# connortannahill/MM-ADMM

Hardware: AMD Instinct MI355X
Metric: ADMM iterations/sec on 1M-node 2D mesh; achieved HBM GB/s in SpMV (higher is better)
Workload: dtype f64

## Files before the change

### include/mmx_sparse.h

```cpp
#ifndef MMX_SPARSE_H
#define MMX_SPARSE_H

#include <stdint.h>

#include "mmadmm.h"

#ifdef __cplusplus
extern "C" {
#endif

typedef struct mmx_param_iter {
  int order;
  int level;
  int drop_ilu;
  int ipiv;
  int iscal;
  int nitmax;
  double resid_reduc;
  int info;
  double drop_tol;
  int new_rhat;
  int iaccel;
  int north;
} mmx_param_iter;

typedef struct mmx_struc_s* mmx_struc;
typedef struct mmx_matrix_s* mmx_matrix;

typedef struct mmx_sparse_stats {
  long long solves, iterations, spmvs, sweeps, factors;
  double t_spmv_ms, t_sweep_ms, t_factor_ms, t_vec_ms, t_solve_ms;
  long long n_spmv_timed, n_sweep_timed, n_factor_timed;
  double spmv_bytes;
  double last_rms, rmsi;
  int sweep_mode;
  int sweep_e;
  int factor_mode;
  int sweep_e_bwd;
} mmx_sparse_stats;

void mmx_param_iter_default(mmx_param_iter* p);
void mmx_param_iter_mesh(mmx_param_iter* p);

int mmx_struc_create(int n, int no_diag, mmx_struc* out);
int mmx_struc_set_entry(mmx_struc s, int row, int col);
int mmx_struc_set_entries(mmx_struc s, long long count, const int32_t* rows, const int32_t* cols);
int mmx_struc_mesh_pattern(mmx_struc s, int dim, int nF, const int32_t* F);
int mmx_struc_pack(mmx_struc s);
int mmx_struc_get(mmx_struc s, int* n, long long* nnz, int32_t* ia, int32_t* ja);
int mmx_struc_destroy(mmx_struc s);

int mmx_matrix_create(int device, int n, const int32_t* ia, const int32_t* ja, mmx_matrix* out);
int mmx_matrix_create_from_struc(int device, mmx_struc s, mmx_matrix* out);
int mmx_matrix_sizes(mmx_matrix m, int* n, long long* nnz);
int mmx_matrix_stream(mmx_matrix m, void** hip_stream);
int mmx_matrix_set_values(mmx_matrix m, const double* a);
int mmx_matrix_set_values_device(mmx_matrix m, const double* d_a);
int mmx_matrix_set_rhs(mmx_matrix m, const double* b);
int mmx_matrix_set_rhs_device(mmx_matrix m, const double* d_b);
int mmx_matrix_set_toler(mmx_matrix m, const double* tol);
int mmx_matrix_sfac(mmx_matrix m, const mmx_param_iter* p);
int mmx_matrix_solve(mmx_matrix m, const mmx_param_iter* p, double* x, int* nitr, int initial_guess);
int mmx_matrix_solve_device(mmx_matrix m, const mmx_param_iter* p, double* d_x, int* nitr, int initial_guess);
int mmx_matrix_matmult(mmx_matrix m, const double* x, double* y);
int mmx_matrix_matmult_device(mmx_matrix m, const double* d_x, double* d_y);
int mmx_matrix_factor(mmx_matrix m);
int mmx_matrix_ilu_solve(mmx_matrix m, const double* b, double* x);
int mmx_matrix_ilu_solve_device(mmx_matrix m, const double* d_b, double* d_x);
int mmx_matrix_factor_nnz(mmx_matrix m, long long* nnzf);
int mmx_matrix_get_factor(mmx_matrix m, int32_t* iaf, int32_t* jaf, double* af, int32_t* diag);
int mmx_matrix_get_scale(mmx_matrix m, double* scal);
int mmx_matrix_set_timing(mmx_matrix m, int on);
int mmx_matrix_stats_get(mmx_matrix m, mmx_sparse_stats* out);
int mmx_matrix_stats_reset(mmx_matrix m);
int mmx_matrix_destroy(mmx_matrix m);

int mmx_ilu_symbolic(int n, const int32_t* ia, const int32_t* ja, int level, long long* nnzf, int32_t* iaf,
                     int32_t* jaf, int32_t* diag);

int mmx_matrix_chain_prof(mmx_matrix m, unsigned long long* out, int reset);
int mmx_sweep_schedule_info(int n, const int32_t* ia, const int32_t* ja, int level, int fwd, long long* info);
int mmx_factor_schedule_info(int n, const int32_t* ia, const int32_t* ja, int level, long long* info);

int mmx_stream_copy(int device, const double* d_src, double* d_dst, long long n, int reps, int variant, double* ms);
int mmx_occupy(int device, int blocks, double ms);
int mmx_occupy_wait(void);

#ifdef __cplusplus
}
#endif
#endif
```

### mm-admm_amd/csrc/host/sparse.cpp

```cpp
#include <omp.h>

#include <algorithm>
#include <chrono>
#include <climits>
#include <cmath>
#include <cstdio>
#include <cstring>
#include <exception>
#include <string>
#include <thread>
#include <queue>
#include <vector>

#include "../../../include/mmx_sparse.h"
#include "../kernels/sparse_kernels.h"
#include "chain_sched.h"
#include "common.h"

namespace mmx {
namespace {

struct PhaseTimer {
  bool on;
  const char* who;
// ... 141 lines not shown
      rl[i][q] = lev[cols[q]];
      lev[cols[q]] = kAbsent;
    }
    if (dgRel[i] < 0) throw Error(MMADMM_ERR_INVALID, "row " + std::to_string(i) + " has no diagonal entry");
  }
  iaf.assign(n + 1, 0);
  for (int i = 0; i < n; ++i) iaf[i + 1] = iaf[i] + (int)rj[i].size();
  jaf.resize(iaf[n]);
  for (int i = 0; i < n; ++i) std::copy(rj[i].begin(), rj[i].end(), jaf.begin() + iaf[i]);
}

namespace {

int spmv_version() {
  static int v = [] {
    const char* e = getenv("MMX_SPMV");
    return (e && atoi(e) == 1) ? 1 : 2;
  }();
  return v;
}

void check_params(const mmx_param_iter& p) {
  if (p.order != 0) throw Error(MMADMM_ERR_INVALID, "unsupported ParamIter.order (only natural ordering, 0)");
  if (p.drop_ilu != 0) throw Error(MMADMM_ERR_INVALID, "unsupported ParamIter.drop_ilu (only level-of-fill ILU, 0)");
  if (p.ipiv != 0) throw Error(MMADMM_ERR_INVALID, "unsupported ParamIter.ipiv (only no pivoting, 0)");
  if (p.iscal != 0 && p.iscal != 1)
    throw Error(MMADMM_ERR_INVALID, "unsupported ParamIter.iscal (0 no scaling, 1 diagonal row scaling)");
  if (p.iaccel != 0 && p.iaccel != 1 && p.iaccel != -1)
    throw Error(MMADMM_ERR_INVALID, "unsupported ParamIter.iaccel (0 CG-STAB, 1 ORTHOMIN, -1 CG)");
  if (p.iaccel == 1 && p.north < 1) throw Error(MMADMM_ERR_INVALID, "ParamIter.north must be >= 1 for ORTHOMIN");
  if (p.level < 0) throw Error(MMADMM_ERR_INVALID, "ParamIter.level must be >= 0");
}

struct Timer {
  hipEvent_t a = nullptr, b = nullptr;
  bool armed = false;
  void init() {
    if (!a) {
      MMX_HIP(hipEventCreateWithFlags(&a, hipEventDisableSystemFence));
      MMX_HIP(hipEventCreateWithFlags(&b, hipEventDisableSystemFence));
    }
  }
  ~Timer() {
    if (a) (void)hipEventDestroy(a);
    if (b) (void)hipEventDestroy(b);
  }
};

}

struct SparseMatrix {
  int device = 0;
  hipStream_t st = nullptr;
  int n = 0;
  long long nnz = 0;
  std::vector<int> ia, ja;
  DevBuf<int> d_ia, d_ja, d_rowblk;
  DevBuf<int4> d_desc;
  int nblk = 0;
  DevBuf<double> d_a, d_b, d_tol;
  bool tolSet = false;
  bool symbolic = false;
  int level = -1;
  std::vector<int> iaf, jaf, dgRel;
  DevBuf<int> d_iaf, d_jaf, d_dg, d_amap, d_permf, d_permb;
  DevBuf<int2> d_piv;
  DevBuf<int> d_toff;
  DevBuf<signed char> d_tgt;
  bool facLds = false;
  int nchf = 0, nchb = 0, nlevf = 0, nlevb = 0;
  DevBuf<double> d_af;
  DevBuf<unsigned> d_flags, d_ctl;
  DevBuf<uint64_t> d_gy, d_gx;
  unsigned epoch = 0, fepoch = 0;
  struct ChainDir {
    int E = 0;
    long long nent = 0, nslot = 0;
    DevBuf<int> bandSlot, bandT, bandImp, bandNImp, bandE, bandOrder, laneStart, laneLen, laneSkew, laneNs, code, src, dsrc,
        impRow, impSlot, impWait, impNeed;
    DevBuf<uint16_t> code16;
    DevBuf<double> val, dval;
    ChainArgs args{};
  };
  ChainDir chf, chb;
  bool useChain = false;
  struct FactorDir {
    DevBuf<int> bandSlot, bandT, laneLen, laneSkew, bandOrder, bandImp, bandNImp, impPos, impCnt, impSlot, impWait,
        impNeed, meta, rowStart, vsrc;
    DevBuf<uint16_t> code;
    DevBuf<double> val, af0;
    DevBuf<uint64_t> gU;
    FactorArgs args{};
// ... 15 lines not shown
  int ominNorth = 0;
  DevBuf<AccelScalars> d_asc;
  AccelScalars* h_asc = nullptr;
  bool timing = false;
  mmx_sparse_stats stats{};
  Timer tm[4];

  SparseMatrix(int dev, int n_, const int* ia_, const int* ja_) : device(dev), n(n_) {
    if (n <= 0) throw Error(MMADMM_ERR_INVALID, "matrix size must be positive");
    if (ia_[0] != 0) throw Error(MMADMM_ERR_INVALID, "ia[0] must be 0");
    for (int i = 0; i < n; ++i)
      if (ia_[i + 1] < ia_[i]) throw Error(MMADMM_ERR_INVALID, "ia must be non-decreasing");
    nnz = ia_[n];
    int bad = 0;
#pragma omp parallel for schedule(static) reduction(max : bad)
    for (long long k = 0; k < nnz; ++k)
      if (ja_[k] < 0 || ja_[k] >= n) bad = 1;
    if (bad) throw Error(MMADMM_ERR_INVALID, "column index out of range");
    ia.assign(ia_, ia_ + n + 1);
    ja.resize(nnz);
#pragma omp parallel for schedule(static)
    for (long long k = 0; k < nnz; ++k) ja[k] = ja_[k];
    int ndev = 0;
    if (hipGetDeviceCount(&ndev) != hipSuccess || ndev == 0) throw Error(MMADMM_ERR_HIP, "no HIP device available");
    MMX_HIP(hipSetDevice(device));
    MMX_HIP(hipStreamCreateWithFlags(&st, hipStreamNonBlocking));
    d_ia.upload(ia.data(), ia.size(), st);
    d_ja.alloc((size_t)nnz + 2);
    if (nnz * sizeof(int) >= ((size_t)16 << 20))
      upload_staged(d_ja.p, ja.data(), (size_t)nnz * sizeof(int), st);
    else if (nnz)
      MMX_HIP(hipMemcpyAsync(d_ja.p, ja.data(), (size_t)nnz * sizeof(int), hipMemcpyHostToDevice, st));
    MMX_HIP(hipMemsetAsync(d_ja.p + nnz, 0, 2 * sizeof(int), st));
    d_a.alloc(nnz + 2);
    MMX_HIP(hipMemsetAsync(d_a.p, 0, sizeof(double) * (nnz + 2), st));
    d_b.alloc(n);
    MMX_HIP(hipMemsetAsync(d_b.p, 0, sizeof(double) * n, st));
    std::vector<int> rb{0};
    int r0 = 0;
    while (r0 < n) {
      int r = r0 + 1;
      while (r < n && ia[r + 1] - ia[r0] <= kSpmvTile && r - r0 < 4 * kSpmvBlock) ++r;
      rb.push_back(r);
      r0 = r;
    }
    nblk = (int)rb.size() - 1;
    d_rowblk.upload(rb.data(), rb.size(), st);
    std::vector<int4> desc(nblk);
    for (int b = 0; b < nblk; ++b) desc[b] = make_int4(rb[b], rb[b + 1], ia[rb[b]], ia[rb[b + 1]]);
    d_desc.upload(desc.data(), desc.size(), st);
    std::vector<int> adiag(n, -1);
    int missing = 0;
#pragma omp parallel for schedule(static) reduction(max : missing)
    for (int i = 0; i < n; ++i) {
      for (int k = ia[i]; k < ia[i + 1]; ++k)
        if (ja[k] == i) {
          adiag[i] = k;
          break;
        }
      if (adiag[i] < 0) missing = 1;
    }
    allDiag = missing == 0;
    d_adiag.upload(adiag.data(), adiag.size(), st);
    MMX_HIP(hipStreamSynchronize(st));
    for (DevBuf<double>* v : {&d_res, &d_res0, &d_p, &d_vbar, &d_avbar, &d_s, &d_z, &d_t, &d_x, &d_tmp}) v->alloc(n);
    d_part.alloc((size_t)std::max(nblk, vec_grid(n)) * 3);
    d_sc.alloc(1);
    MMX_HIP(hipMemsetAsync(d_sc.p, 0, sizeof(CgsScalars), st));
    MMX_HIP(hipHostMalloc((void**)&h_sc, sizeof(CgsScalars), hipHostMallocDefault));
    d_asc.alloc(1);
    MMX_HIP(hipMemsetAsync(d_asc.p, 0, sizeof(AccelScalars), st));
    MMX_HIP(hipHostMalloc((void**)&h_asc, sizeof(AccelScalars), hipHostMallocDefault));
    d_ctl.alloc(16);
    MMX_HIP(hipMemsetAsync(d_ctl.p, 0, 16 * sizeof(unsigned), st));
    d_gy.alloc(2 * (size_t)n);
    d_gx.alloc(2 * (size_t)n);
    MMX_HIP(hipMemsetAsync(d_gy.p, 0, 16 * (size_t)n, st));
    MMX_HIP(hipMemsetAsync(d_gx.p, 0, 16 * (size_t)n, st));
    d_flags.alloc(n);
    MMX_HIP(hipMemsetAsync(d_flags.p, 0, sizeof(unsigned) * n, st));
    stats.spmv_bytes = 12.0 * (double)nnz + 4.0 * (n + 1) + 16.0 * n;
    MMX_HIP(hipStreamSynchronize(st));
  }
  ~SparseMatrix() {
    if (st) (void)hipStreamSynchronize(st);
    if (evSpin) (void)hipEventDestroy(evSpin);
    if (h_sc) (void)hipHostFree(h_sc);
    if (h_asc) (void)hipHostFree(h_asc);
    if (st) (void)hipStreamDestroy(st);
  }

  hipEvent_t evSpin = nullptr;
  void spin_sync() {
    static const bool spin = [] {
      const char* e = getenv("MMX_SPIN");
      return !(e && atoi(e) == 0);
    }();
    if (!spin) {
      MMX_HIP(hipStreamSynchronize(st));
      return;
    }
    if (!evSpin) MMX_HIP(hipEventCreateWithFlags(&evSpin, hipEventDisableTiming));
    MMX_HIP(hipEventRecord(evSpin, st));
    hipError_t r;
    while ((r = hipEventQuery(evSpin)) == hipErrorNotReady) __builtin_ia32_pause();
    MMX_HIP(r);
  }

  unsigned* tickets() { return d_ctl.p; }
  unsigned* errw() { return d_ctl.p + 8; }

  void sfac(const mmx_param_iter& p) {
    check_params(p);
    PhaseTimer pt("sfac");
    symbolic_ilu(n, ia, ja, p.level, iaf, jaf, dgRel);
    pt.mark("symbolic");
// ... 388 lines not shown

  void ilu_apply(int pro, const double* src, double* p, double* out, unsigned* tk) {
    begin(1);
    const unsigned ey = next_epoch();
    if (useChain)
      launch_chain_sweep(true, pro, chf.E, chf.args, src, p, d_res.p, d_avbar.p, d_sc.p, nullptr, d_gy.p, nullptr, ey,
                         tk, errw(), st);
    else
      launch_sweep(true, pro, d_iaf.p, d_jaf.p, d_dg.p, d_af.p, d_permf.p, nchf, src, p, d_res.p, d_avbar.p, d_sc.p,
                   nullptr, d_gy.p, nullptr, ey, tk, errw(), st);
    const unsigned ex = next_epoch();
    const char* bg = getenv("MMX_BWD_GRAN");
    const bool fromGran = !(bg && atoi(bg) == 0);
    if (useChain) {
      launch_chain_sweep(false, 0, chb.E, chb.args, nullptr, nullptr, nullptr, nullptr, nullptr, d_gy.p, d_gx.p,
                         fromGran ? nullptr : out, ex, tk + 1, errw(), st);
      if (fromGran) launch_gran_extract(n, d_gx.p, out, st);
    } else
      launch_sweep(false, 0, d_iaf.p, d_jaf.p, d_dg.p, d_af.p, d_permb.p, nchb, nullptr, nullptr, nullptr, nullptr,
                   nullptr, d_gy.p, d_gx.p, out, ex, tk + 1, errw(), st);
    MMX_HIP(hipGetLastError());
    const float ms = end(1);
    stats.sweeps += 2;
    if (timing) {
      stats.t_sweep_ms += ms;
      stats.n_sweep_timed += 2;
    }
  }

  void spmv(int epi, const double* x, double* y, const double* e1) {
    begin(0);
    if (spmv_version() == 1)
      launch_spmv(epi, nblk, d_rowblk.p, d_ia.p, d_ja.p, d_a.p, x, y, e1, d_part.p, st);
    else
      launch_spmv2(epi, nblk, d_desc.p, d_ia.p, d_ja.p, d_a.p, x, y, e1, d_part.p, st);
    MMX_HIP(hipGetLastError());
    const float ms = end(0);
    stats.spmvs++;
    if (timing) {
      stats.t_spmv_ms += ms;
      stats.n_spmv_timed++;
    }
  }

  void scale_rows() {
    if (!allDiag) throw Error(MMADMM_ERR_INVALID, "ParamIter.iscal = 1 needs a diagonal entry in every row");
    if (!d_ascal.p) d_ascal.alloc(n);
    launch_scale_rows(nblk, d_desc.p, d_ia.p, d_adiag.p, d_a.p, d_b.p, d_ascal.p, st);
    MMX_HIP(hipGetLastError());
    scaled = true;
    if (scaledVersion != valVersion) {
      scaledVersion = valVersion;
      factVersion = -1;
    }
  }

  void omin_buffers(int north) {
    if (ominNorth == north) return;
    ominNorth = 0;
    try {
      d_oq.alloc((size_t)north * n);
      d_oaq.alloc((size_t)north * n);
      d_oms.alloc(2 * (size_t)north);
      d_opart.alloc((size_t)std::max(north, 2) * vec_grid(n));
    } catch (...) {
      (void)hipGetLastError();
      d_oq.alloc(0);
      d_oaq.alloc(0);
// ... 508 lines not shown
  return guarded([&] {
    MMX_M(m);
    if (!M.symbolic) throw Error(MMADMM_ERR_INVALID, "no symbolic factor (call mmx_matrix_sfac)");
    if (iaf) std::memcpy(iaf, M.iaf.data(), sizeof(int) * (M.n + 1));
    if (jaf) std::memcpy(jaf, M.jaf.data(), sizeof(int) * M.jaf.size());
    if (diag) std::memcpy(diag, M.dgRel.data(), sizeof(int) * M.n);
    if (af) {
      MMX_HIP(hipMemcpyAsync(af, M.d_af.p, sizeof(double) * M.jaf.size(), hipMemcpyDeviceToHost, M.st));
      MMX_HIP(hipStreamSynchronize(M.st));
    }
  });
}

int mmx_matrix_get_scale(mmx_matrix m, double* scal) {
  return guarded([&] {
    MMX_M(m);
    if (!scal) throw Error(MMADMM_ERR_INVALID, "bad arguments");
    if (!M.scaled) {
      std::fill(scal, scal + M.n, 1.0);
      return;
    }
    MMX_HIP(hipMemcpyAsync(scal, M.d_ascal.p, sizeof(double) * M.n, hipMemcpyDeviceToHost, M.st));
    MMX_HIP(hipStreamSynchronize(M.st));
  });
}

int mmx_matrix_set_timing(mmx_matrix m, int on) {
  return guarded([&] {
    MMX_M(m);
    M.timing = on != 0;
  });
}

int mmx_matrix_stats_get(mmx_matrix m, mmx_sparse_stats* out) {
  return guarded([&] {
    MMX_M(m);
    if (out) {
      *out = M.stats;
      out->sweep_mode = M.useChain ? 1 : 0;
      out->factor_mode = M.useChainFactor ? 1 : M.facWave ? 2 : 0;
      out->sweep_e = M.useChain ? M.chf.E : 0;
      out->sweep_e_bwd = M.useChain ? M.chb.E : 0;
    }
  });
}

int mmx_matrix_chain_prof(mmx_matrix m, unsigned long long* out, int reset) {
  return guarded([&] {
    MMX_M(m);
    if (!M.d_cprof.p) throw Error(MMADMM_ERR_INVALID, "chain profiling off (set MMX_CHAIN_PROF=1 before sfac)");
    if (out)
      MMX_HIP(hipMemcpyAsync(out, M.d_cprof.p, 1024 * sizeof(unsigned long long), hipMemcpyDeviceToHost, M.st));
    if (reset) MMX_HIP(hipMemsetAsync(M.d_cprof.p, 0, 1024 * sizeof(unsigned long long), M.st));
    MMX_HIP(hipStreamSynchronize(M.st));
  });
}

int mmx_matrix_stats_reset(mmx_matrix m) {
  return guarded([&] {
    MMX_M(m);
    const double bytes = M.stats.spmv_bytes;
    M.stats = mmx_sparse_stats{};
    M.stats.spmv_bytes = bytes;
  });
}

int mmx_ilu_symbolic(int n, const int32_t* ia, const int32_t* ja, int level, long long* nnzf, int32_t* iaf,
                     int32_t* jaf, int32_t* diag) {
  return guarded([&] {
    if (n <= 0 || !ia || !ja || level < 0) throw Error(MMADMM_ERR_INVALID, "bad arguments");
    std::vector<int> via(ia, ia + n + 1), vja(ja, ja + ia[n]), fia, fja, dg;
    mmx::symbolic_ilu(n, via, vja, level, fia, fja, dg);
    if (nnzf) *nnzf = (long long)fja.size();
    if (iaf) std::memcpy(iaf, fia.data(), sizeof(int) * (n + 1));
    if (jaf) std::memcpy(jaf, fja.data(), sizeof(int) * fja.size());
// ... 107 lines not shown
```

### mm-admm_amd/csrc/kernels/layout.h

```cpp
#pragma once

#ifndef MMX_ZU_INTER
#define MMX_ZU_INTER 0
#endif
#ifndef MMX_SPMV_TILE
#define MMX_SPMV_TILE 2048
#endif
#ifndef MMX_SPMV_BLOCK
#define MMX_SPMV_BLOCK 256
#endif
#ifndef MMX_B3_PAIRS
#define MMX_B3_PAIRS 1
#endif
#ifndef MMX_CHAIN_VEC
#define MMX_CHAIN_VEC 1
#endif
#ifndef MMX_CHAIN_CODE16
#define MMX_CHAIN_CODE16 1
#endif

namespace mmx {
constexpr unsigned kLayoutPartials = 6;
constexpr unsigned kLayoutBkinvBlock = 64;
constexpr unsigned kLayoutWord = 0x4d000000u | ((unsigned)(MMX_ZU_INTER != 0) << 0) |
                                 ((unsigned)(MMX_CHAIN_VEC != 0) << 1) | ((unsigned)(MMX_CHAIN_CODE16 != 0) << 2) |
                                 (((unsigned)MMX_SPMV_TILE / 256u & 0xFu) << 4) |
                                 (((unsigned)MMX_SPMV_BLOCK / 64u & 0xFu) << 8) | ((kLayoutPartials & 0xFu) << 12) |
                                 ((kLayoutBkinvBlock / 64u & 0x3u) << 16) | ((unsigned)(MMX_B3_PAIRS != 0) << 18);
}
```

### mm-admm_amd/csrc/kernels/sparse_kernels.h

```cpp
#pragma once
#include <hip/hip_runtime.h>
#include <stdint.h>

#include "layout.h"

namespace mmx {

constexpr int kSpmvTile = MMX_SPMV_TILE;
constexpr int kSpmvBlock = MMX_SPMV_BLOCK;
constexpr int kSweepRows = 64;
constexpr int kSweepGrid = 128;
constexpr int kVecBlock = 256;
int vec_grid(int n);

struct CgsScalars {
  double rho, rholst, alpha, omega, beta, rmsi, rms, ctol, iconv;
  int conv;
  int pad;
};

struct SweepCtl {
  unsigned* tickets;
  unsigned* err;
};

void launch_spmv(int epi, int nblk, const int* rowblk, const int* ia, const int* ja, const double* a,
                 const double* x, double* y, const double* e1, double* partials, hipStream_t st);
void launch_spmv2(int epi, int nblk, const int4* desc, const int* ia, const int* ja, const double* a,
                  const double* x, double* y, const double* e1, double* partials, hipStream_t st);

void launch_ilu_factor(const int* ia, const int* ja, const double* a, const int* amap, const int* iaf, const int* jaf,
                       const int* dg, const int2* piv, const int* perm, int nchunks, double* af, unsigned* flags,
                       unsigned epoch, unsigned* ticket, unsigned* err, hipStream_t st);

constexpr int kFacW = 127;
void launch_ilu_factor_lds(const int* ia, const double* a, const int* amap, const int* iaf, const int* jaf, const int* dg,
                           const int2* piv, const int* toff, const signed char* tgt, const int* perm, int nchunks,
                           double* af, unsigned* flags, unsigned epoch, unsigned* ticket, unsigned* err, hipStream_t st);

constexpr int kFacWaveNL = 32;
void launch_ilu_factor_wave(const int* ia, const double* a, const int* amap, const int* iaf, const int* dg,
                            const int2* piv, const int* jaf, const int* toff, const signed char* tgt, const int* perm,
                            int nrows, double* af, unsigned* flags, uint64_t* gF, unsigned epoch, unsigned* ticket,
                            unsigned* err, hipStream_t st);
void launch_fac_prep(int n, const int* iaf, const int* jaf, const int* dg, const long long* rowTot, int2* piv,
                     int* toff, signed char* tgt, hipStream_t st);
void launch_occupy(int blocks, double ms, double* sink, hipStream_t st);

void launch_sweep(bool fwd, int pro, const int* iaf, const int* jaf, const int* dg, const double* af, const int* perm,
                  int nchunks, const double* src, double* p, const double* res, const double* avbar, const CgsScalars* sc,
                  const uint64_t* gin, uint64_t* gout, double* out, unsigned epoch, unsigned* ticket, unsigned* err,
                  hipStream_t st);

inline constexpr bool chain_code16(int ee) { return MMX_CHAIN_CODE16 || ee > 32; }

struct ChainArgs {
  const int* bandSlot;
  const int* bandT;
  const int* bandImp;
  const int* bandNImp;
  const int* laneStart;
  const int* laneLen;
// ... 84 lines not shown
```

### mm-admm_amd/csrc/kernels/sparse_kernels.hip

```cpp
#include <hip/hip_runtime.h>

#include <algorithm>

#include <cstdlib>

#include "block_reduce.h"
#include "sparse_kernels.h"

namespace mmx {

namespace {

constexpr unsigned kSpinMax = 1u << 24;
constexpr int kBatch = 4;
constexpr int kFactorBatch = 8;

__device__ __forceinline__ void store_granule(uint64_t* g, unsigned epoch, double v) {
  const uint64_t bits = (uint64_t)__double_as_longlong(v);
  const uint64_t tag = (uint64_t)epoch << 32;
  __hip_atomic_store(g, tag | (bits & 0xffffffffull), __ATOMIC_RELAXED, __HIP_MEMORY_SCOPE_AGENT);
  __hip_atomic_store(g + 1, tag | (bits >> 32), __ATOMIC_RELAXED, __HIP_MEMORY_SCOPE_AGENT);
}

__device__ __forceinline__ bool load_granule(const uint64_t* g, unsigned epoch, double& v) {
// ... 73 lines not shown
        pv[1] += s * s;
      }
    }
  } else {
    double s = 0.0;
    for (int c = k0; c < k1; c += kSpmvTile) {
      const int ce = (c + kSpmvTile < k1) ? c + kSpmvTile : k1;
      for (int k = c + (int)threadIdx.x; k < ce; k += kSpmvBlock) prod[k - c] = a[k] * x[ja[k]];
      __syncthreads();
      if (threadIdx.x == 0)
        for (int k = c; k < ce; ++k) s += prod[k - c];
      __syncthreads();
    }
    if (threadIdx.x == 0) {
      y[r0] = s;
      if (EPI == 1) pv[0] += e1[r0] * s;
      if (EPI == 2) {
        pv[0] += s * e1[r0];
        pv[1] += s * s;
      }
    }
  }
  if (EPI != 0) {
    __syncthreads();
    block_sum<2, kSpmvBlock>(pv, red);
    if (threadIdx.x == 0) {
      partials[(size_t)b * 2 + 0] = pv[0];
      partials[(size_t)b * 2 + 1] = pv[1];
    }
  }
}

constexpr int kSpmvPairs = kSpmvTile / (2 * kSpmvBlock) + 1;
typedef int v2i_t __attribute__((ext_vector_type(2)));
typedef double v2d_t __attribute__((ext_vector_type(2)));

template <int EPI>
__global__ void __launch_bounds__(kSpmvBlock) k_spmv2(const int4* __restrict__ desc, int nblk,
                                                       const int* __restrict__ ia, const int* __restrict__ ja,
                                                       const double* __restrict__ a, const double* __restrict__ x,
                                                       double* __restrict__ y, const double* __restrict__ e1,
                                                       double* __restrict__ partials) {
  __shared__ double prod[kSpmvTile + 2];
  __shared__ double red[kSpmvBlock][2];
  const int G = (int)gridDim.x;
  const int b = (int)(blockIdx.x % 8) * (G / 8) + (int)(blockIdx.x / 8);
  if (b >= nblk) return;
  const int tid = (int)threadIdx.x;
  const int4 d = desc[b];
  const int r0 = d.x, r1 = d.y, k0 = d.z, k1 = d.w;
  double pv[2] = {0.0, 0.0};
  if (k1 - k0 <= kSpmvTile) {
    const int ka = k0 & ~1;
    const int np = (k1 - ka + 1) >> 1;
    const int rf = r0 + tid;
    const int rc = rf < r1 ? rf : r1 - 1;
    int ib = ia[rc], ie = ia[rc + 1];
    double ef = 0.0;
    if (EPI != 0) ef = e1[rc];
    const int pmax = np > 0 ? np - 1 : 0;
    v2i_t jv[kSpmvPairs];
    v2d_t av[kSpmvPairs];
#pragma unroll
    for (int j = 0; j < kSpmvPairs; ++j) {
      const int p = min(tid + j * kSpmvBlock, pmax);
      jv[j] = __builtin_nontemporal_load(reinterpret_cast<const v2i_t*>(ja + ka) + p);
      av[j] = __builtin_nontemporal_load(reinterpret_cast<const v2d_t*>(a + ka) + p);
    }
    double xv0[kSpmvPairs], xv1[kSpmvPairs];
#pragma unroll
    for (int j = 0; j < kSpmvPairs; ++j) {
      xv0[j] = x[jv[j].x];
      xv1[j] = x[jv[j].y];
    }
#pragma unroll
    for (int j = 0; j < kSpmvPairs; ++j) {
      const int p = tid + j * kSpmvBlock;
      if (p < np) {
        prod[2 * p] = av[j].x * xv0[j];
        prod[2 * p + 1] = av[j].y * xv1[j];
      }
    }
    __syncthreads();
    for (int r = rf; r < r1; r += kSpmvBlock) {
      if (r != rf) {
        ib = ia[r];
        ie = ia[r + 1];
        if (EPI != 0) ef = e1[r];
      }
      double s = 0.0;
      for (int kk = ib; kk < ie; ++kk) s += prod[kk - ka];
      y[r] = s;
      if (EPI == 1) pv[0] += ef * s;
      if (EPI == 2) {
        pv[0] += s * ef;
        pv[1] += s * s;
      }
    }
  } else {
    double s = 0.0;
    for (int c = k0; c < k1; c += kSpmvTile) {
      const int ce = (c + kSpmvTile < k1) ? c + kSpmvTile : k1;
      for (int k = c + tid; k < ce; k += kSpmvBlock) prod[k - c] = a[k] * x[ja[k]];
      __syncthreads();
      if (tid == 0)
        for (int k = c; k < ce; ++k) s += prod[k - c];
      __syncthreads();
    }
    if (tid == 0) {
      y[r0] = s;
      if (EPI == 1) pv[0] += e1[r0] * s;
      if (EPI == 2) {
        pv[0] += s * e1[r0];
        pv[1] += s * s;
      }
// ... 535 lines not shown
    sc->rho = rho;
    sc->beta = beta;
    sc->rholst = rho;
    sc->conv = 0;
  } else if (MODE == 1) {
    sc->alpha = sc->rho / v[0];
  } else if (MODE == 2) {
    sc->omega = v[0] / (v[1] + tiny);
  } else {
    const double rms = sqrt(v[0]);
    sc->rms = rms;
    sc->iconv = v[2];
    sc->conv = (v[2] == 0.0 || (rms / sc->rmsi) < sc->ctol) ? 1 : 0;
    const double rho = v[1];
    double beta = rho / (sc->rholst + tiny);
    beta *= (sc->alpha / (sc->omega + tiny));
    sc->rho = rho;
    sc->beta = beta;
    sc->rholst = rho;
  }
}

void launch_spmv(int epi, int nblk, const int* rowblk, const int* ia, const int* ja, const double* a, const double* x,
                 double* y, const double* e1, double* partials, hipStream_t st) {
  if (nblk <= 0) return;
  if (epi == 0)
    hipLaunchKernelGGL(k_spmv<0>, dim3(nblk), dim3(kSpmvBlock), 0, st, rowblk, ia, ja, a, x, y, e1, partials);
  else if (epi == 1)
    hipLaunchKernelGGL(k_spmv<1>, dim3(nblk), dim3(kSpmvBlock), 0, st, rowblk, ia, ja, a, x, y, e1, partials);
  else
    hipLaunchKernelGGL(k_spmv<2>, dim3(nblk), dim3(kSpmvBlock), 0, st, rowblk, ia, ja, a, x, y, e1, partials);
}

void launch_spmv2(int epi, int nblk, const int4* desc, const int* ia, const int* ja, const double* a, const double* x,
                  double* y, const double* e1, double* partials, hipStream_t st) {
  if (nblk <= 0) return;
  const dim3 g((unsigned)((nblk + 7) / 8 * 8)), bl(kSpmvBlock);
  if (epi == 0)
    hipLaunchKernelGGL(k_spmv2<0>, g, bl, 0, st, desc, nblk, ia, ja, a, x, y, e1, partials);
  else if (epi == 1)
    hipLaunchKernelGGL(k_spmv2<1>, g, bl, 0, st, desc, nblk, ia, ja, a, x, y, e1, partials);
  else
    hipLaunchKernelGGL(k_spmv2<2>, g, bl, 0, st, desc, nblk, ia, ja, a, x, y, e1, partials);
}

void launch_ilu_factor_lds(const int* ia, const double* a, const int* amap, const int* iaf, const int* jaf, const int* dg,
                           const int2* piv, const int* toff, const signed char* tgt, const int* perm, int nchunks,
                           double* af, unsigned* flags, unsigned epoch, unsigned* ticket, unsigned* err, hipStream_t st) {
  if (nchunks <= 0) return;
  const int grid = nchunks < sweep_grid() ? nchunks : sweep_grid();
  hipLaunchKernelGGL((k_ilu_factor_lds<8, 8>), dim3(grid), dim3(kSweepRows), 0, st, ia, a, amap, iaf, jaf, dg, piv, toff,
                     tgt, perm, nchunks, af, flags, epoch, ticket, err);
}

constexpr int kFacWaveChunk = 0;
static int factor_wg() {
  static const int v = [] {
    const char* e = getenv("MMX_FAC_WG");
    return (e && atoi(e) == 8) ? 8 : 4;
  }();
  return v;
}
int ilu_factor_wave_grid() {
  static int g = [] {
    int dev = 0, cus = 0, nb = 0, nb2 = 0;
    (void)hipGetDevice(&dev);
    (void)hipDeviceGetAttribute(&cus, hipDeviceAttributeMultiprocessorCount, dev);
    if (factor_wg() == 8) {
      (void)hipOccupancyMaxActiveBlocksPerMultiprocessor(&nb, k_ilu_factor_wave<kFacWaveNL, true, 8>, 512, 0);
      (void)hipOccupancyMaxActiveBlocksPerMultiprocessor(&nb2, k_ilu_factor_wave<kFacWaveNL, false, 8>, 512, 0);
    } else {
      (void)hipOccupancyMaxActiveBlocksPerMultiprocessor(&nb, k_ilu_factor_wave<kFacWaveNL, true>, 256, 0);
      (void)hipOccupancyMaxActiveBlocksPerMultiprocessor(&nb2, k_ilu_factor_wave<kFacWaveNL, false>, 256, 0);
    }
    nb = nb < nb2 ? nb : nb2;
    nb = nb < 1 ? 1 : (nb > 8 ? 8 : nb);
// ... 234 lines not shown
```

### mm-admm_amd/python/lasolver_amd.py

```python
import ctypes

import numpy as np

from mmadmm_amd import MMADMMError, _check, c_double_p, c_int_p, lib as _mlib

_cfg = False


class ParamIter(ctypes.Structure):
    _fields_ = [("order", ctypes.c_int), ("level", ctypes.c_int), ("drop_ilu", ctypes.c_int),
                ("ipiv", ctypes.c_int), ("iscal", ctypes.c_int), ("nitmax", ctypes.c_int),
                ("resid_reduc", ctypes.c_double), ("info", ctypes.c_int), ("drop_tol", ctypes.c_double),
                ("new_rhat", ctypes.c_int), ("iaccel", ctypes.c_int), ("north", ctypes.c_int)]

    def __init__(self):
        super().__init__()
        lib().mmx_param_iter_default(ctypes.byref(self))

    @staticmethod
    def mesh():
        p = ParamIter()
        lib().mmx_param_iter_mesh(ctypes.byref(p))
        return p


class SparseStats(ctypes.Structure):
    _fields_ = [("solves", ctypes.c_longlong), ("iterations", ctypes.c_longlong), ("spmvs", ctypes.c_longlong),
                ("sweeps", ctypes.c_longlong), ("factors", ctypes.c_longlong), ("t_spmv_ms", ctypes.c_double),
                ("t_sweep_ms", ctypes.c_double), ("t_factor_ms", ctypes.c_double), ("t_vec_ms", ctypes.c_double),
                ("t_solve_ms", ctypes.c_double), ("n_spmv_timed", ctypes.c_longlong),
                ("n_sweep_timed", ctypes.c_longlong), ("n_factor_timed", ctypes.c_longlong),
                ("spmv_bytes", ctypes.c_double), ("last_rms", ctypes.c_double), ("rmsi", ctypes.c_double),
                ("sweep_mode", ctypes.c_int), ("sweep_e", ctypes.c_int), ("factor_mode", ctypes.c_int),
                ("sweep_e_bwd", ctypes.c_int)]

    def as_dict(self):
        return {k: getattr(self, k) for k, _ in self._fields_}


def lib():
    global _cfg
    L = _mlib()
    if _cfg:
        return L
    vp, i, ll, d = ctypes.c_void_p, ctypes.c_int, ctypes.c_longlong, ctypes.c_double
    pp = ctypes.POINTER(ParamIter)
    L.mmx_param_iter_default.argtypes = [pp]
    L.mmx_param_iter_default.restype = None
    L.mmx_param_iter_mesh.argtypes = [pp]
    L.mmx_param_iter_mesh.restype = None
    L.mmx_struc_create.argtypes = [i, i, ctypes.POINTER(vp)]
    L.mmx_struc_set_entry.argtypes = [vp, i, i]
    L.mmx_struc_set_entries.argtypes = [vp, ll, c_int_p, c_int_p]
    L.mmx_struc_mesh_pattern.argtypes = [vp, i, i, c_int_p]
    L.mmx_struc_pack.argtypes = [vp]
    L.mmx_struc_get.argtypes = [vp, ctypes.POINTER(i), ctypes.POINTER(ll), c_int_p, c_int_p]
    L.mmx_struc_destroy.argtypes = [vp]
    L.mmx_matrix_create.argtypes = [i, i, c_int_p, c_int_p, ctypes.POINTER(vp)]
    L.mmx_matrix_create_from_struc.argtypes = [i, vp, ctypes.POINTER(vp)]
    L.mmx_matrix_sizes.argtypes = [vp, ctypes.POINTER(i), ctypes.POINTER(ll)]
    L.mmx_matrix_stream.argtypes = [vp, ctypes.POINTER(vp)]
    L.mmx_matrix_set_values.argtypes = [vp, c_double_p]
    L.mmx_matrix_set_values_device.argtypes = [vp, vp]
    L.mmx_matrix_set_rhs.argtypes = [vp, c_double_p]
    L.mmx_matrix_set_rhs_device.argtypes = [vp, vp]
    L.mmx_matrix_set_toler.argtypes = [vp, c_double_p]
    L.mmx_matrix_sfac.argtypes = [vp, pp]
    L.mmx_matrix_solve.argtypes = [vp, pp, c_double_p, ctypes.POINTER(i), i]
    L.mmx_matrix_solve_device.argtypes = [vp, pp, vp, ctypes.POINTER(i), i]
    L.mmx_matrix_matmult.argtypes = [vp, c_double_p, c_double_p]
    L.mmx_matrix_matmult_device.argtypes = [vp, vp, vp]
    L.mmx_matrix_factor.argtypes = [vp]
    L.mmx_matrix_ilu_solve.argtypes = [vp, c_double_p, c_double_p]
    L.mmx_matrix_ilu_solve_device.argtypes = [vp, vp, vp]
    L.mmx_matrix_factor_nnz.argtypes = [vp, ctypes.POINTER(ll)]
    L.mmx_matrix_get_factor.argtypes = [vp, c_int_p, c_int_p, c_double_p, c_int_p]
    L.mmx_matrix_get_scale.argtypes = [vp, c_double_p]
    L.mmx_matrix_set_timing.argtypes = [vp, i]
    L.mmx_matrix_stats_get.argtypes = [vp, ctypes.POINTER(SparseStats)]
    L.mmx_matrix_stats_reset.argtypes = [vp]
    L.mmx_matrix_destroy.argtypes = [vp]
    L.mmx_stream_copy.argtypes = [i, vp, vp, ll, i, i, ctypes.POINTER(ctypes.c_double)]
    L.mmx_occupy.argtypes = [i, i, ctypes.c_double]
    L.mmx_occupy_wait.argtypes = []
    L.mmx_ilu_symbolic.argtypes = [i, c_int_p, c_int_p, i, ctypes.POINTER(ll), c_int_p, c_int_p, c_int_p]
    _cfg = True
    return L


def _i32(a):
    return np.ascontiguousarray(a, dtype=np.int32)


def _f64(a):
    return np.ascontiguousarray(a, dtype=np.float64)


class MatrixStruc:

    def __init__(self, n, no_diag=0):
        self.h = ctypes.c_void_p()
        _check(lib().mmx_struc_create(int(n), int(no_diag), ctypes.byref(self.h)))
        self.n = int(n)

    def set_entry(self, row, col):
        _check(lib().mmx_struc_set_entry(self.h, int(row), int(col)))

    def set_entries(self, rows, cols):
        rows, cols = _i32(rows), _i32(cols)
        if rows.shape != cols.shape:
            raise ValueError("rows and cols differ in length")
# ... 100 lines not shown
    def get_factor(self):
        nz = ctypes.c_longlong()
        _check(lib().mmx_matrix_factor_nnz(self.h, ctypes.byref(nz)))
        iaf = np.zeros(self.n + 1, np.int32)
        jaf = np.zeros(nz.value, np.int32)
        af = np.zeros(nz.value)
        dg = np.zeros(self.n, np.int32)
        _check(lib().mmx_matrix_get_factor(self.h, iaf.ctypes.data_as(c_int_p), jaf.ctypes.data_as(c_int_p),
                                           af.ctypes.data_as(c_double_p), dg.ctypes.data_as(c_int_p)))
        return iaf, jaf, af, dg

    def set_values_device(self, ptr):
        _check(lib().mmx_matrix_set_values_device(self.h, ctypes.c_void_p(ptr)))

    def set_rhs_device(self, ptr):
        _check(lib().mmx_matrix_set_rhs_device(self.h, ctypes.c_void_p(ptr)))

    def matmult_device(self, xptr, yptr):
        _check(lib().mmx_matrix_matmult_device(self.h, ctypes.c_void_p(xptr), ctypes.c_void_p(yptr)))

    def solve_device(self, param, xptr, initial_guess=0):
        if param.iaccel == -1:
            param.iscal = 0
        nitr = ctypes.c_int()
        _check(lib().mmx_matrix_solve_device(self.h, ctypes.byref(param), ctypes.c_void_p(xptr),
                                             ctypes.byref(nitr), int(initial_guess)))
        return nitr.value

    def stream(self):
        s = ctypes.c_void_p()
        _check(lib().mmx_matrix_stream(self.h, ctypes.byref(s)))
        return s.value

    def set_timing(self, on=True):
        _check(lib().mmx_matrix_set_timing(self.h, 1 if on else 0))

    def stats(self):
        s = SparseStats()
        _check(lib().mmx_matrix_stats_get(self.h, ctypes.byref(s)))
        return s.as_dict()

    def reset_stats(self):
        _check(lib().mmx_matrix_stats_reset(self.h))

    def close(self):
        if lib is None:
            return
        if getattr(self, "h", None) and self.h.value:
            lib().mmx_matrix_destroy(self.h)
            self.h = ctypes.c_void_p()

    def __del__(self):
        self.close()


def ilu_symbolic(ia, ja, level):
    ia, ja = _i32(ia), _i32(ja)
    n = len(ia) - 1
    nz = ctypes.c_longlong()
    _check(lib().mmx_ilu_symbolic(n, ia.ctypes.data_as(c_int_p), ja.ctypes.data_as(c_int_p), int(level),
                                  ctypes.byref(nz), None, None, None))
    iaf = np.zeros(n + 1, np.int32)
    jaf = np.zeros(nz.value, np.int32)
    dg = np.zeros(n, np.int32)
    _check(lib().mmx_ilu_symbolic(n, ia.ctypes.data_as(c_int_p), ja.ctypes.data_as(c_int_p), int(level), None,
                                  iaf.ctypes.data_as(c_int_p), jaf.ctypes.data_as(c_int_p), dg.ctypes.data_as(c_int_p)))
# ... 24 lines not shown
```

Measured before the change: 2655.

## Compress SpMV column indices using detected contiguous block groups

At matrix creation the code checks whether the CSR pattern consists of aligned contiguous column groups of 3 or 2 (as in vector-valued mesh systems). When such groups are found, it stores one index per group and the SpMV kernel rebuilds the column indices, or loads x as 2-wide vectors for groups of 2. This cuts index traffic from 4 bytes per nonzero to 4/G bytes. For groups of 3 it adds per-element integer divides and still issues two scattered index loads per pair, and matrix creation gains a detection pass and an extra device buffer.

```diff
diff --git a/include/mmx_sparse.h b/include/mmx_sparse.h
--- a/include/mmx_sparse.h
+++ b/include/mmx_sparse.h
@@ -37,6 +37,8 @@
   int sweep_e;
   int factor_mode;
   int sweep_e_bwd;
+  int spmv_group;
+  double spmv_bytes_moved;
 } mmx_sparse_stats;
 
 void mmx_param_iter_default(mmx_param_iter* p);
@@ -70,6 +72,7 @@
 int mmx_matrix_factor_nnz(mmx_matrix m, long long* nnzf);
 int mmx_matrix_get_factor(mmx_matrix m, int32_t* iaf, int32_t* jaf, double* af, int32_t* diag);
 int mmx_matrix_get_scale(mmx_matrix m, double* scal);
+int mmx_matrix_set_spmv_mode(mmx_matrix m, int mode);
 int mmx_matrix_set_timing(mmx_matrix m, int on);
 int mmx_matrix_stats_get(mmx_matrix m, mmx_sparse_stats* out);
 int mmx_matrix_stats_reset(mmx_matrix m);
diff --git a/mm-admm_amd/csrc/host/sparse.cpp b/mm-admm_amd/csrc/host/sparse.cpp
--- a/mm-admm_amd/csrc/host/sparse.cpp
+++ b/mm-admm_amd/csrc/host/sparse.cpp
@@ -197,6 +197,30 @@
   if (p.level < 0) throw Error(MMADMM_ERR_INVALID, "ParamIter.level must be >= 0");
 }
 
+int detect_groups(int n, long long nnz, const std::vector<int>& ia, const std::vector<int>& ja, std::vector<int>& jg) {
+  for (int G : {3, 2}) {
+    if (n % G != 0 || nnz % G != 0 || nnz == 0) continue;
+    int bad = 0;
+#pragma omp parallel for schedule(static) reduction(max : bad)
+    for (int r = 0; r <= n; ++r)
+      if (ia[r] % G != 0) bad = 1;
+    if (bad) continue;
+    const long long ng = nnz / G;
+    jg.resize((size_t)ng);
+#pragma omp parallel for schedule(static) reduction(max : bad)
+    for (long long g = 0; g < ng; ++g) {
+      const int c0 = ja[(size_t)g * G];
+      int b = c0 % G != 0;
+      for (int c = 1; c < G; ++c) b |= ja[(size_t)g * G + c] != c0 + c;
+      if (b) bad = 1;
+      jg[(size_t)g] = c0 / G;
+    }
+    if (!bad) return G;
+  }
+  jg.clear();
+  return 0;
+}
+
 struct Timer {
   hipEvent_t a = nullptr, b = nullptr;
   bool armed = false;
@@ -223,6 +247,8 @@
   DevBuf<int> d_ia, d_ja, d_rowblk;
   DevBuf<int4> d_desc;
   int nblk = 0;
+  int spmvGroup = 0, spmvMode = 1;
+  DevBuf<int> d_jg;
   DevBuf<double> d_a, d_b, d_tol;
   bool tolSet = false;
   bool symbolic = false;
@@ -304,6 +330,22 @@
     else if (nnz)
       MMX_HIP(hipMemcpyAsync(d_ja.p, ja.data(), (size_t)nnz * sizeof(int), hipMemcpyHostToDevice, st));
     MMX_HIP(hipMemsetAsync(d_ja.p + nnz, 0, 2 * sizeof(int), st));
+    {
+      PhaseTimer pt("matrix create");
+      std::vector<int> jg;
+      spmvGroup = detect_groups(n, nnz, ia, ja, jg);
+      if (spmvGroup) {
+        const size_t ng = (size_t)(nnz / spmvGroup);
+        d_jg.alloc(ng + MMX_SPMV_JG_PAD);
+        if (ng * sizeof(int) >= ((size_t)16 << 20))
+          upload_staged(d_jg.p, jg.data(), ng * sizeof(int), st);
+        else if (ng)
+          MMX_HIP(hipMemcpyAsync(d_jg.p, jg.data(), ng * sizeof(int), hipMemcpyHostToDevice, st));
+        MMX_HIP(hipMemsetAsync(d_jg.p + ng, 0, MMX_SPMV_JG_PAD * sizeof(int), st));
+        MMX_HIP(hipStreamSynchronize(st));
+      }
+      pt.mark(spmvGroup == 3 ? "spmv groups of 3" : spmvGroup == 2 ? "spmv groups of 2" : "spmv groups (none)");
+    }
     d_a.alloc(nnz + 2);
     MMX_HIP(hipMemsetAsync(d_a.p, 0, sizeof(double) * (nnz + 2), st));
     d_b.alloc(n);
@@ -354,6 +396,7 @@
     stats.spmv_bytes = 12.0 * (double)nnz + 4.0 * (n + 1) + 16.0 * n;
     MMX_HIP(hipStreamSynchronize(st));
   }
+  int spmv_group() const { return (spmvMode == 1 && spmv_version() != 1) ? spmvGroup : 0; }
   ~SparseMatrix() {
     if (st) (void)hipStreamSynchronize(st);
     if (evSpin) (void)hipEventDestroy(evSpin);
@@ -808,8 +851,11 @@
     begin(0);
     if (spmv_version() == 1)
       launch_spmv(epi, nblk, d_rowblk.p, d_ia.p, d_ja.p, d_a.p, x, y, e1, d_part.p, st);
-    else
-      launch_spmv2(epi, nblk, d_desc.p, d_ia.p, d_ja.p, d_a.p, x, y, e1, d_part.p, st);
+    else {
+      int grp = spmv_group();
+      if (grp == 2 && (reinterpret_cast<uintptr_t>(x) & 15) != 0) grp = 0;
+      launch_spmv2(epi, grp, nblk, d_desc.p, d_ia.p, d_ja.p, d_jg.p, d_a.p, x, y, e1, d_part.p, st);
+    }
     MMX_HIP(hipGetLastError());
     const float ms = end(0);
     stats.spmvs++;
@@ -1384,6 +1430,14 @@
   });
 }
 
+int mmx_matrix_set_spmv_mode(mmx_matrix m, int mode) {
+  return guarded([&] {
+    MMX_M(m);
+    if (mode != 0 && mode != 1) throw Error(MMADMM_ERR_INVALID, "mmx_matrix_set_spmv_mode: mode must be 0 or 1");
+    M.spmvMode = mode;
+  });
+}
+
 int mmx_matrix_stats_get(mmx_matrix m, mmx_sparse_stats* out) {
   return guarded([&] {
     MMX_M(m);
@@ -1393,6 +1447,10 @@
       out->factor_mode = M.useChainFactor ? 1 : M.facWave ? 2 : 0;
       out->sweep_e = M.useChain ? M.chf.E : 0;
       out->sweep_e_bwd = M.useChain ? M.chb.E : 0;
+      const int G = M.spmv_group();
+      out->spmv_group = G;
+      out->spmv_bytes_moved = (G ? 8.0 * (double)M.nnz + 4.0 * (double)(M.nnz / G) : 12.0 * (double)M.nnz) +
+                              4.0 * (M.n + 1) + 16.0 * M.n;
     }
   });
 }
diff --git a/mm-admm_amd/csrc/kernels/layout.h b/mm-admm_amd/csrc/kernels/layout.h
--- a/mm-admm_amd/csrc/kernels/layout.h
+++ b/mm-admm_amd/csrc/kernels/layout.h
@@ -8,6 +8,9 @@
 #endif
 #ifndef MMX_SPMV_BLOCK
 #define MMX_SPMV_BLOCK 256
+#endif
+#ifndef MMX_SPMV_JG_PAD
+#define MMX_SPMV_JG_PAD 2
 #endif
 #ifndef MMX_B3_PAIRS
 #define MMX_B3_PAIRS 1
@@ -26,5 +29,6 @@
                                  ((unsigned)(MMX_CHAIN_VEC != 0) << 1) | ((unsigned)(MMX_CHAIN_CODE16 != 0) << 2) |
                                  (((unsigned)MMX_SPMV_TILE / 256u & 0xFu) << 4) |
                                  (((unsigned)MMX_SPMV_BLOCK / 64u & 0xFu) << 8) | ((kLayoutPartials & 0xFu) << 12) |
-                                 ((kLayoutBkinvBlock / 64u & 0x3u) << 16) | ((unsigned)(MMX_B3_PAIRS != 0) << 18);
+                                 ((kLayoutBkinvBlock / 64u & 0x3u) << 16) | ((unsigned)(MMX_B3_PAIRS != 0) << 18) |
+                                 (((unsigned)MMX_SPMV_JG_PAD & 0x3u) << 19);
 }
diff --git a/mm-admm_amd/csrc/kernels/sparse_kernels.h b/mm-admm_amd/csrc/kernels/sparse_kernels.h
--- a/mm-admm_amd/csrc/kernels/sparse_kernels.h
+++ b/mm-admm_amd/csrc/kernels/sparse_kernels.h
@@ -26,8 +26,8 @@
 
 void launch_spmv(int epi, int nblk, const int* rowblk, const int* ia, const int* ja, const double* a,
                  const double* x, double* y, const double* e1, double* partials, hipStream_t st);
-void launch_spmv2(int epi, int nblk, const int4* desc, const int* ia, const int* ja, const double* a,
-                  const double* x, double* y, const double* e1, double* partials, hipStream_t st);
+void launch_spmv2(int epi, int grp, int nblk, const int4* desc, const int* ia, const int* ja, const int* jg,
+                  const double* a, const double* x, double* y, const double* e1, double* partials, hipStream_t st);
 
 void launch_ilu_factor(const int* ia, const int* ja, const double* a, const int* amap, const int* iaf, const int* jaf,
                        const int* dg, const int2* piv, const int* perm, int nchunks, double* af, unsigned* flags,
diff --git a/mm-admm_amd/csrc/kernels/sparse_kernels.hip b/mm-admm_amd/csrc/kernels/sparse_kernels.hip
--- a/mm-admm_amd/csrc/kernels/sparse_kernels.hip
+++ b/mm-admm_amd/csrc/kernels/sparse_kernels.hip
@@ -129,16 +129,80 @@
 }
 
 constexpr int kSpmvPairs = kSpmvTile / (2 * kSpmvBlock) + 1;
+constexpr int kSpmvGroups2 = kSpmvTile / (2 * kSpmvBlock);
 typedef int v2i_t __attribute__((ext_vector_type(2)));
 typedef double v2d_t __attribute__((ext_vector_type(2)));
+
+template <int GRP>
+__device__ __forceinline__ void spmv2_products(const int* __restrict__ ja, const int* __restrict__ jg,
+                                               const double* __restrict__ a, const double* __restrict__ x, int k0,
+                                               int k1, int tid, double* prod) {
+  if (GRP == 2) {
+    const int ng = (k1 - k0) >> 1;
+    const int gmax = ng > 0 ? ng - 1 : 0;
+    const int* jt = jg + (k0 >> 1);
+    const v2d_t* at = reinterpret_cast<const v2d_t*>(a + k0);
+    int jv[kSpmvGroups2];
+    v2d_t av[kSpmvGroups2], xv[kSpmvGroups2];
+#pragma unroll
+    for (int j = 0; j < kSpmvGroups2; ++j) {
+      const int g = min(tid + j * kSpmvBlock, gmax);
+      jv[j] = __builtin_nontemporal_load(jt + g);
+      av[j] = __builtin_nontemporal_load(at + g);
+    }
+#pragma unroll
+    for (int j = 0; j < kSpmvGroups2; ++j) xv[j] = reinterpret_cast<const v2d_t*>(x)[jv[j]];
+#pragma unroll
+    for (int j = 0; j < kSpmvGroups2; ++j) {
+      const int g = tid + j * kSpmvBlock;
+      if (g < ng) {
+        prod[2 * g] = av[j].x * xv[j].x;
+        prod[2 * g + 1] = av[j].y * xv[j].y;
+      }
+    }
+    return;
+  }
+  const int ka = k0 & ~1;
+  const int np = (k1 - ka + 1) >> 1;
+  const int pmax = np > 0 ? np - 1 : 0;
+  v2i_t jv[kSpmvPairs];
+  v2d_t av[kSpmvPairs];
+#pragma unroll
+  for (int j = 0; j < kSpmvPairs; ++j) {
+    const int p = min(tid + j * kSpmvBlock, pmax);
+    if (GRP == 3) {
+      const int e = ka + 2 * p, q0 = e / 3, q1 = (e + 1) / 3;
+      jv[j].x = 3 * __builtin_nontemporal_load(jg + q0) + (e - 3 * q0);
+      jv[j].y = 3 * __builtin_nontemporal_load(jg + q1) + (e + 1 - 3 * q1);
+    } else {
+      jv[j] = __builtin_nontemporal_load(reinterpret_cast<const v2i_t*>(ja + ka) + p);
+    }
+    av[j] = __builtin_nontemporal_load(reinterpret_cast<const v2d_t*>(a + ka) + p);
+  }
+  double xv0[kSpmvPairs], xv1[kSpmvPairs];
+#pragma unroll
+  for (int j = 0; j < kSpmvPairs; ++j) {
+    xv0[j] = x[jv[j].x];
+    xv1[j] = x[jv[j].y];
+  }
+#pragma unroll
+  for (int j = 0; j < kSpmvPairs; ++j) {
+    const int p = tid + j * kSpmvBlock;
+    if (p < np) {
+      prod[2 * p] = av[j].x * xv0[j];
+      prod[2 * p + 1] = av[j].y * xv1[j];
+    }
+  }
+}
 
 template <int EPI>
 __global__ void __launch_bounds__(kSpmvBlock) k_spmv2(const int4* __restrict__ desc, int nblk,
                                                        const int* __restrict__ ia, const int* __restrict__ ja,
                                                        const double* __restrict__ a, const double* __restrict__ x,
                                                        double* __restrict__ y, const double* __restrict__ e1,
-                                                       double* __restrict__ partials) {
-  __shared__ double prod[kSpmvTile + 2];
+                                                       double* __restrict__ partials, const int* __restrict__ jg,
+                                                       int grp) {
+  __shared__ __attribute__((aligned(16))) double prod[kSpmvTile + 2];
   __shared__ double red[kSpmvBlock][2];
   const int G = (int)gridDim.x;
   const int b = (int)(blockIdx.x % 8) * (G / 8) + (int)(blockIdx.x / 8);
@@ -149,35 +213,17 @@
   double pv[2] = {0.0, 0.0};
   if (k1 - k0 <= kSpmvTile) {
     const int ka = k0 & ~1;
-    const int np = (k1 - ka + 1) >> 1;
     const int rf = r0 + tid;
     const int rc = rf < r1 ? rf : r1 - 1;
     int ib = ia[rc], ie = ia[rc + 1];
     double ef = 0.0;
     if (EPI != 0) ef = e1[rc];
-    const int pmax = np > 0 ? np - 1 : 0;
-    v2i_t jv[kSpmvPairs];
-    v2d_t av[kSpmvPairs];
-#pragma unroll
-    for (int j = 0; j < kSpmvPairs; ++j) {
-      const int p = min(tid + j * kSpmvBlock, pmax);
-      jv[j] = __builtin_nontemporal_load(reinterpret_cast<const v2i_t*>(ja + ka) + p);
-      av[j] = __builtin_nontemporal_load(reinterpret_cast<const v2d_t*>(a + ka) + p);
-    }
-    double xv0[kSpmvPairs], xv1[kSpmvPairs];
-#pragma unroll
-    for (int j = 0; j < kSpmvPairs; ++j) {
-      xv0[j] = x[jv[j].x];
-      xv1[j] = x[jv[j].y];
-    }
-#pragma unroll
-    for (int j = 0; j < kSpmvPairs; ++j) {
-      const int p = tid + j * kSpmvBlock;
-      if (p < np) {
-        prod[2 * p] = av[j].x * xv0[j];
-        prod[2 * p + 1] = av[j].y * xv1[j];
-      }
-    }
+    if (grp == 2)
+      spmv2_products<2>(ja, jg, a, x, k0, k1, tid, prod);
+    else if (grp == 3)
+      spmv2_products<3>(ja, jg, a, x, k0, k1, tid, prod);
+    else
+      spmv2_products<0>(ja, jg, a, x, k0, k1, tid, prod);
     __syncthreads();
     for (int r = rf; r < r1; r += kSpmvBlock) {
       if (r != rf) {
@@ -779,16 +825,16 @@
     hipLaunchKernelGGL(k_spmv<2>, dim3(nblk), dim3(kSpmvBlock), 0, st, rowblk, ia, ja, a, x, y, e1, partials);
 }
 
-void launch_spmv2(int epi, int nblk, const int4* desc, const int* ia, const int* ja, const double* a, const double* x,
-                  double* y, const double* e1, double* partials, hipStream_t st) {
+void launch_spmv2(int epi, int grp, int nblk, const int4* desc, const int* ia, const int* ja, const int* jg,
+                  const double* a, const double* x, double* y, const double* e1, double* partials, hipStream_t st) {
   if (nblk <= 0) return;
   const dim3 g((unsigned)((nblk + 7) / 8 * 8)), bl(kSpmvBlock);
   if (epi == 0)
-    hipLaunchKernelGGL(k_spmv2<0>, g, bl, 0, st, desc, nblk, ia, ja, a, x, y, e1, partials);
+    hipLaunchKernelGGL(k_spmv2<0>, g, bl, 0, st, desc, nblk, ia, ja, a, x, y, e1, partials, jg, grp);
   else if (epi == 1)
-    hipLaunchKernelGGL(k_spmv2<1>, g, bl, 0, st, desc, nblk, ia, ja, a, x, y, e1, partials);
+    hipLaunchKernelGGL(k_spmv2<1>, g, bl, 0, st, desc, nblk, ia, ja, a, x, y, e1, partials, jg, grp);
   else
-    hipLaunchKernelGGL(k_spmv2<2>, g, bl, 0, st, desc, nblk, ia, ja, a, x, y, e1, partials);
+    hipLaunchKernelGGL(k_spmv2<2>, g, bl, 0, st, desc, nblk, ia, ja, a, x, y, e1, partials, jg, grp);
 }
 
 void launch_ilu_factor_lds(const int* ia, const double* a, const int* amap, const int* iaf, const int* jaf, const int* dg,
diff --git a/mm-admm_amd/python/lasolver_amd.py b/mm-admm_amd/python/lasolver_amd.py
--- a/mm-admm_amd/python/lasolver_amd.py
+++ b/mm-admm_amd/python/lasolver_amd.py
@@ -32,7 +32,7 @@
                 ("n_sweep_timed", ctypes.c_longlong), ("n_factor_timed", ctypes.c_longlong),
                 ("spmv_bytes", ctypes.c_double), ("last_rms", ctypes.c_double), ("rmsi", ctypes.c_double),
                 ("sweep_mode", ctypes.c_int), ("sweep_e", ctypes.c_int), ("factor_mode", ctypes.c_int),
-                ("sweep_e_bwd", ctypes.c_int)]
+                ("sweep_e_bwd", ctypes.c_int), ("spmv_group", ctypes.c_int), ("spmv_bytes_moved", ctypes.c_double)]
 
     def as_dict(self):
         return {k: getattr(self, k) for k, _ in self._fields_}
@@ -77,6 +77,7 @@
     L.mmx_matrix_get_factor.argtypes = [vp, c_int_p, c_int_p, c_double_p, c_int_p]
     L.mmx_matrix_get_scale.argtypes = [vp, c_double_p]
     L.mmx_matrix_set_timing.argtypes = [vp, i]
+    L.mmx_matrix_set_spmv_mode.argtypes = [vp, i]
     L.mmx_matrix_stats_get.argtypes = [vp, ctypes.POINTER(SparseStats)]
     L.mmx_matrix_stats_reset.argtypes = [vp]
     L.mmx_matrix_destroy.argtypes = [vp]
@@ -243,6 +244,9 @@
         _check(lib().mmx_matrix_stream(self.h, ctypes.byref(s)))
         return s.value
 
+    def set_spmv_mode(self, mode):
+        _check(lib().mmx_matrix_set_spmv_mode(self.h, int(mode)))
+
     def set_timing(self, on=True):
         _check(lib().mmx_matrix_set_timing(self.h, 1 if on else 0))
 
diff --git a/profiles/r08/spmv_grouped/spmv_modes.py b/profiles/r08/spmv_grouped/spmv_modes.py
--- /dev/null
+++ b/profiles/r08/spmv_grouped/spmv_modes.py
@@ -0,0 +1,51 @@
+import json
+import os
+import sys
+
+ROOT = os.path.dirname(os.path.dirname(os.path.dirname(os.path.dirname(os.path.abspath(__file__)))))
+sys.path.insert(0, os.path.join(ROOT, "mm-admm_amd", "python"))
+import numpy as np
+import torch
+import lasolver_amd as la
+import mmadmm_amd as mx
+
+dim, nn = (3, 63) if "--3d" in sys.argv else (2, 707)
+modes = [int(m) for m in sys.argv[1:] if m.lstrip("-").isdigit()] or [None]
+mesh = mx.MeshData.rect(dim, nn)
+s = la.MatrixStruc(dim * mesh.nP)
+s.mesh_pattern(dim, mesh.F)
+s.pack()
+n = s.n
+nnz = s.getnja()
+rng = np.random.default_rng(20221015)
+a = rng.uniform(-1.0, 1.0, nnz)
+x = rng.uniform(-1.0, 1.0, n)
+A = la.MatrixIter(s)
+A.a[:] = a
+A.upload()
+xd = torch.from_numpy(x).cuda()
+yd = torch.empty(n, dtype=torch.float64, device="cuda")
+torch.cuda.synchronize()
+ref = None
+for rnd in range(3 if modes != [None] else 1):
+    for m in modes:
+        if m is not None:
+            A.set_spmv_mode(m)
+        A.set_timing(False)
+        for _ in range(5):
+            A.matmult_device(xd.data_ptr(), yd.data_ptr())
+        A.set_timing(True)
+        A.reset_stats()
+        for _ in range(50):
+            A.matmult_device(xd.data_ptr(), yd.data_ptr())
+        st = A.stats()
+        torch.cuda.synchronize()
+        y = yd.cpu().numpy()
+        if ref is None:
+            ref = y.copy()
+        ms = st["t_spmv_ms"] / st["n_spmv_timed"]
+        print(json.dumps({"dim": dim, "n": n, "nnz": nnz, "mode": m, "round": rnd, "avg_ms": round(ms, 5),
+                          "spmv_group": st.get("spmv_group"), "bytes_moved": st.get("spmv_bytes_moved"),
+                          "bytes_alg": st["spmv_bytes"], "alg_GBs": round(st["spmv_bytes"] / ms / 1e6, 1),
+                          "bit_equal_first": bool(np.array_equal(y, ref))}), flush=True)
+A.close()
```

Result: no change. 2655 (median of 2 runs) (+0.0%).
